# CristianSimion5/vk-raytracing-engine

Measured on AMD Instinct MI355X. Metric: Mrays/s, higher is better.
Workload: dtype f32

## Files before the change

### vk-raytracing-engine_amd/csrc/device_scene.h

```cpp
#pragma once
#include <hip/hip_runtime.h>
#include <stddef.h>
#include <stdint.h>
#include "../../include/vkrt_host_device.h"
#include "device_math.h"

struct DevInstance
{
  float o2w[12];
  float w2o[9];
  int32_t primMesh;
  uint32_t vis;
  int32_t pad;
};
static_assert(sizeof(DevInstance) == 96, "DevInstance");
#define VKRT_VIS_CULL_DISABLE 0x100u
#define VKRT_VIS_FLIP 0x200u
#define VKRT_VIS_MIRRORED 0x10000u

#define VKRT_VERTEX_QUADS 3
#define VKRT_VERTEX_BYTES 48u
struct DevTexRef
{
  uint32_t offset;
// ... 118 lines not shown
  uint32_t tilesX, tileCount;
  uint32_t tileFirst;
  float* image;
  unsigned int* workCounter;
  DevCounters* counters;
};

struct WfBuffers
{
  unsigned* ctrl;
  float4* planes;
  float4* stage;
  uint32_t capacity;
  uint32_t groups;
  float4* sampleState;
};
```

### vk-raytracing-engine_amd/csrc/kernels.h

```cpp
#pragma once
#include <hip/hip_runtime.h>
#include "device_scene.h"
#include "wf_schedule.h"

hipError_t vkrt_launch_pathtrace(const TraceParams& P, unsigned gridBlocks, bool count, hipStream_t stream);
int        vkrt_pathtrace_block_size();
hipError_t vkrt_pathtrace_occupancy(size_t ldsBytes, int* blocksPerCU);
hipError_t vkrt_launch_trace_rays(const DevScene& sc, unsigned n, const float* o, const float* d, float tmin, float tmax, int anyHit,
                                  float* t, float* u, float* v, int* gid, hipStream_t stream);
hipError_t vkrt_launch_eval_math(int op, unsigned n, const float* a, const float* b, float* out, hipStream_t stream);
#define VKRT_EVAL_SHADE_MAX_LIGHTS 16
hipError_t vkrt_launch_eval_shade(unsigned n, const float* in, float4* lights, float* out, hipStream_t stream);

hipError_t vkrt_launch_query(const DevQueryScene& sc, const float4* rays, uint64_t n, uint32_t seed, bool filter, bool opaque, bool alpha, float4* hits,
                             int* occ, hipStream_t stream);
hipError_t vkrt_launch_query_multi(const DevQueryScene& sc, const float4* rays, uint64_t n, uint32_t seed, bool filter, bool opaque, bool alpha,
                                   uint32_t maxHits, float4* hits, int* counts, hipStream_t stream);
hipError_t vkrt_launch_closest_point(const DevQueryScene& sc, const float4* queries, uint64_t n, bool filter, float4* hits, unsigned long long* work,
                                     hipStream_t stream);
hipError_t vkrt_launch_node_masks(const DevScene& sc, uint32_t nodeCount, uint32_t instCount, uint32_t sweeps, uint2* masks, hipStream_t stream);
hipError_t vkrt_launch_material_alpha(DevMaterial* table, uint32_t first, uint32_t count, const uint2* src, hipStream_t stream);
hipError_t vkrt_launch_hit_surface(const DevSurfaceScene& sc, const float4* hits, uint32_t n, bool material, float4* out, hipStream_t stream);

struct WfTiming
{
  hipEvent_t* events;
  int capacity;
  int used;
};
struct WfAsync
{
  hipStream_t streams[VKRT_WF_MAX_LANES];
  hipEvent_t fork, join[VKRT_WF_MAX_LANES];
  int count;
  hipEvent_t* pool;
  int poolSize;
};
size_t     vkrt_wf_state_bytes(uint32_t pathCapacity, int groups);
void       vkrt_wf_carve(void* base, uint32_t pathCapacity, int groups, WfBuffers* B);
struct WfOptions
{
  int subframes;
  int travBlock;
  int inFlight;
};
hipError_t vkrt_launch_wavefront(const TraceParams& P, const WfBuffers& B, const WfOptions& opt, int frames, uint32_t seedStep, bool count,
                                 hipStream_t stream, WfTiming* timing, const WfAsync* async);
void       vkrt_wf_launch_traverse(const TraceParams& P, const WfBuffers& B, int r, unsigned travBlock, bool count, dim3 tg, size_t tlds,
                                   hipStream_t stream);
void       vkrt_wf_launch_traverse_camera(const TraceParams& P, const WfBuffers& B, int r, int smpl, bool count, size_t tlds, hipStream_t stream);

struct HybridGi
{
  float4* color;
// ... 54 lines not shown
```

### vk-raytracing-engine_amd/csrc/vkrt_api.cpp

```cpp
#include <hip/hip_runtime.h>

#include <algorithm>
#include <chrono>
#include <cmath>
#include <cstdarg>
#include <cstdio>
#include <cstdlib>
#include <cstring>
#include <initializer_list>
#include <string>
#include <vector>

#include "../../include/vkrt.h"
#include "bvh_host.h"
#include "dev_buffer.h"
#include "device_scene.h"
#include "kernels.h"
#include "wide_node.h"

#define VKRT_TRI_THRESHOLD_DEFAULT 32
#define VKRT_WF_SHARE_DEFAULT 16
#define VKRT_WF_SHARE_FLAGS_DEFAULT 25
#define VKRT_WF_FRAMES_IN_FLIGHT_DEFAULT 3
#define VKRT_SPLIT_BUDGET_DEFAULT -1
// ... 37 lines not shown
  std::vector<uint32_t> indices;
  std::vector<vkrt_prim_mesh> primMeshes;
  std::vector<vkrt_node> nodes;
  uint32_t lightCount = 0, materialCount = 0;
  std::vector<float> materialAlpha;
  std::vector<void*> allocs;
  DevScene dev{};
  vkrt::TreeBuffers accel;
  bool built = false;
  vkrt_accel_info info{};
  unsigned int* workCounter = nullptr;
  DevCounters* counters = nullptr;
  hipEvent_t evStart = nullptr, evStop = nullptr;
  bool timed = false;
  void* wfMem = nullptr;
  WfBuffers wf{};
  WfAsync wfAsync{};
  std::vector<hipEvent_t> wfEvents;
  WfTiming wfTiming{};
  bool wfTimed = false;
  int splitResolved = 0;
  int wfTimingRounds = 0;
  std::vector<hipEvent_t> wfPool;
  int opt[VKRT_OPT_ALPHA_TEST + 1] = {0, 1, 1, 3, 64, VKRT_WF_SHARE_DEFAULT, VKRT_TRI_THRESHOLD_DEFAULT, 0, VKRT_WF_SHARE_FLAGS_DEFAULT, 1, 0, 0, 0,
                                            VKRT_WF_FRAMES_IN_FLIGHT_DEFAULT, VKRT_SPLIT_BUDGET_DEFAULT, VKRT_WF_SAMPLE_SYNC_DEFAULT, VKRT_WF_CAMERA_ROUNDS_DEFAULT,
                                      VKRT_WF_TRI_LEND_DEFAULT, 0};
  bool hasLargeTriangles = false;
  bool wavefront = true;
  bool stale = false;
  bool refitted = false;
// ... 212 lines not shown
{
  groups = std::max(1, std::min(VKRT_WF_MAX_LANES, groups));
  if(paths >= (1u << 28))
    return fail(VKRT_ERR_UNSUPPORTED, "wavefront mode: %u path records in one shard (limit 2^28 - 1: split the launch into shards)", paths);
  if(!s->wfMem || s->wf.capacity < paths || (int)s->wf.groups < groups)
  {
    HIP_TRY(hipStreamSynchronize(stream));
    if(s->wfMem) (void)hipFree(s->wfMem);
    s->wfMem = nullptr;
    paths = std::max(paths, s->wf.capacity);
    groups = std::max(groups, (int)s->wf.groups);
    s->wf = WfBuffers{};
    HIP_TRY(hipMalloc(&s->wfMem, vkrt_wf_state_bytes(paths, groups)));
    vkrt_wf_carve(s->wfMem, paths, groups, &s->wf);
  }
  if(s->wfAsync.count == 0)
  {
    HIP_TRY(hipEventCreateWithFlags(&s->wfAsync.fork, hipEventDisableTiming));
    for(int j = 0; j < VKRT_WF_MAX_LANES; j++)
    {
      HIP_TRY(hipStreamCreateWithFlags(&s->wfAsync.streams[j], hipStreamNonBlocking));
      HIP_TRY(hipEventCreateWithFlags(&s->wfAsync.join[j], hipEventDisableTiming));
    }
    s->wfAsync.count = VKRT_WF_MAX_LANES;
  }
  return VKRT_OK;
}

int ensureFrameCall(vkrt_scene* s, uint32_t tiles, uint32_t frames, hipStream_t stream)
{
// ... 432 lines not shown
  if(hipEventCreate(&s->evStart) != hipSuccess || hipEventCreate(&s->evStop) != hipSuccess)
    return bail(fail(VKRT_ERR_HIP, "hipEventCreate"));
  *out = s;
  return VKRT_OK;
}

void vkrt_scene_destroy(vkrt_scene* s)
{
  if(!s)
    return;
  (void)hipSetDevice(s->device);
  freeAccel(s);
  for(void* p : s->allocs)
    (void)hipFree(p);
  if(s->wfMem) (void)hipFree(s->wfMem);
  if(s->wfAsync.count)
  {
    (void)hipEventDestroy(s->wfAsync.fork);
    for(int j = 0; j < s->wfAsync.count; j++)
    {
      (void)hipStreamDestroy(s->wfAsync.streams[j]);
      (void)hipEventDestroy(s->wfAsync.join[j]);
    }
  }
  for(hipEvent_t e : s->wfEvents) (void)hipEventDestroy(e);
  for(hipEvent_t e : s->wfPool) (void)hipEventDestroy(e);
  if(s->evStart) (void)hipEventDestroy(s->evStart);
  if(s->evStop) (void)hipEventDestroy(s->evStop);
  delete s;
}
// ... 1431 lines not shown
```

### vk-raytracing-engine_amd/csrc/wavefront.hip

```cpp
#include <hip/hip_runtime.h>
#include <algorithm>
#include <cstdlib>
#include <cstring>

#include "device_math.h"
#include "device_scene.h"
#include "kernels.h"
#include "rgen.h"
#include "hybrid_gi.h"
#include "shade.h"
#include "traverse.h"
#include "traverse_wide.h"
#include "traverse_share.h"

#define WF_BLOCK 256
#define VKRT_FLAG_COUNT_WORK 2u

#include "wf_streams.h"

VKRT_DEV unsigned packFlags(const LaneState& L)
{
  return (L.prd.depth & 0xffu) | (((unsigned)L.smpl & 0xffffu) << 8) | ((L.prd.isSpecular ? 1u : 0u) << 25);
}

VKRT_DEV void loadCommon(const TraceParams& P, const WfBuffers& B, int parity, int type, unsigned i, LaneState& L)
{
  const float4 s0 = wfLoad(rec(B, parity, type, WF_S0, i)), s1 = wfLoad(rec(B, parity, type, WF_S1, i)), s2 = wfLoad(rec(B, parity, type, WF_S2, i));
  const unsigned flags = __float_as_uint(s1.w), pix = __float_as_uint(s2.w);
  L.curWeight = mk3(s0.x, s0.y, s0.z); L.prd.seed = __float_as_uint(s0.w);
  L.hitValue = mk3(s1.x, s1.y, s1.z);
  L.prd.depth = flags & 0xffu; L.smpl = (int)((flags >> 8) & 0xffffu);
  L.prd.isSpecular = ((flags >> 25) & 1u) != 0u;
  L.hitValues = mk3(s2.x, s2.y, s2.z);
// ... 33 lines not shown
VKRT_DEV int finishSegment(const TraceParams& P, const WfBuffers& B, LaneState& L, bool shadowHit, f3 contrib, f3 nextWeight)
{
  const SegmentStep step = stepSegment(P, L, shadowHit, contrib, nextWeight);
  if(step == SEG_SAMPLE_END)
  {
    if(P.flags & VKRT_FLAG_SAMPLE_SYNC)
    {
      wfStore(B.sampleState + pixelSlot(P, L.px, L.lrow), make_float4(L.hitValues.x, L.hitValues.y, L.hitValues.z, __uint_as_float(L.prd.seed)));
      return -1;
    }
    startSample(P, L);
  }
  return step == SEG_PIXEL_DONE ? -1 : WF_C;
}

VKRT_DEV unsigned claimSlots(const WfBuffers& B, int parity, int to, unsigned lane, unsigned* wsum)
{
  const unsigned wave = threadIdx.x >> 6, nw = blockDim.x >> 6;
  const unsigned long long m[WF_TYPES] = {__ballot(to == WF_C), __ballot(to == WF_S), __ballot(to == WF_P)};
  if(lane == 0)
  {
#pragma unroll
    for(int t = 0; t < WF_TYPES; t++) wsum[t * (nw + 1) + wave] = (unsigned)__popcll(m[t]);
  }
  __syncthreads();
  if(threadIdx.x < WF_TYPES)
  {
    unsigned* w = wsum + threadIdx.x * (nw + 1);
    unsigned tot = 0;
    for(unsigned k = 0; k < nw; k++)
    {
      const unsigned c = w[k];
      w[k] = tot;
      tot += c;
    }
    w[nw] = tot ? atomicAdd(countOf(B, parity, (int)threadIdx.x), tot) : 0u;
  }
  __syncthreads();
  if(to < 0)
    return 0u;
  const unsigned long long below = (1ull << lane) - 1ull;
  const unsigned long long mine = to == WF_C ? m[0] : to == WF_S ? m[1] : m[2];
  return wsum[to * (nw + 1) + nw] + wsum[to * (nw + 1) + wave] + (unsigned)__popcll(mine & below);
}

__global__ __launch_bounds__(WF_BLOCK) void k_wf_init(const TraceParams P, const WfBuffers B)
{
  const unsigned lane = lane_id();
  const unsigned w = blockIdx.x * blockDim.x + threadIdx.x;
  bool alive = false;
  unsigned nPixels = 0;
  LaneState L;
  uint32_t x, y, lrow;
  if(pixelOfWork(P, w, P.tileFirst, x, y, lrow))
  {
    startPixel(P, L, x, y, lrow);
    nPixels = 1;
    if(P.pc.samples <= 0 || P.pc.depth <= 0)
      storePixel(P, L);
    else
      alive = true;
  }
  __shared__ unsigned wsum[WF_TYPES * (WF_BLOCK / 64 + 1)];
  const unsigned slot = claimSlots(B, 0, alive ? WF_C : -1, lane, wsum);
  if(alive)
    storeClosest(B, 0, slot, L);
  __shared__ unsigned long long red[VKRT_COUNTER_STRIDE * (WF_BLOCK / 64)];
  const unsigned vals[6] = {0, 0, 0, 0, 0, nPixels};
  blockAddCounters(&P.counters->v[blockIdx.x % VKRT_COUNTER_SLOTS][0], vals, 6, red);
}

__global__ __launch_bounds__(WF_BLOCK) void k_wf_sample_init(const TraceParams P, const WfBuffers B, const int round, const int smpl)
{
  const unsigned lane = lane_id();
  const unsigned w = blockIdx.x * blockDim.x + threadIdx.x;
  bool alive = false;
  LaneState L;
  uint32_t x, y, lrow;
  if(pixelOfWork(P, w, P.tileFirst, x, y, lrow))
  {
    const float4 st = wfLoad(B.sampleState + pixelSlot(P, x, lrow));
    bindPixel(P, L, x, lrow);
    L.prd.seed = __float_as_uint(st.w);
    L.hitValues = mk3(st.x, st.y, st.z);
    L.smpl = smpl;
    startSample(P, L);
    alive = true;
  }
  __shared__ unsigned wsum[WF_TYPES * (WF_BLOCK / 64 + 1)];
  const unsigned slot = claimSlots(B, round & 1, alive ? WF_C : -1, lane, wsum);
  if(alive)
    storeClosest(B, round & 1, slot, L);
}

VKRT_DEV bool advanceSegmentHybrid(const TraceParams& P, const HybridGi& G, LaneState& L, bool shadowHit, f3 contrib, f3 nextWeight, float lightDist)
{
  L.stage = 0;
  if(giSegmentStep(P.pc, L.prd, L.curWeight, L.hitValue, L.hitValues.x, shadowHit, contrib, nextWeight, lightDist))
    return true;
  hybridStorePixel(P, G, (size_t)L.lrow * P.fullW + L.px, true, L.hitValue, L.hitValues.x, L.hitValues.y);
  return false;
}

struct ShadeLds
{
  float lut[512];
  unsigned wsum[WF_TYPES * (WF_BLOCK / 64 + 1)];
};

template <bool PAIR, bool HYBRID, bool CAMERA = false>
VKRT_DEV void shadeHitBlock(const TraceParams& P, const WfBuffers& B, const HybridGi& G, const int par, const unsigned count, const unsigned block, ShadeLds& lds,
                            const int smpl = 0)
{
  const int type = PAIR ? WF_P : WF_C;
  const unsigned lane = lane_id();
  const unsigned qi = block * WF_BLOCK + threadIdx.x;
  ShadeStats st = shadeStatsInit(P.sc, lds.lut);
  unsigned* wsum = lds.wsum;
  int to = -1;
  LaneState L;
  f3 contrib = mk3(0.0f), nextWeight = mk3(0.0f);
  uint32_t x = 0, y = 0, lrow = 0;
  if(CAMERA ? pixelOfWork(P, qi, P.tileFirst, x, y, lrow) : qi < count)
  {
    if(CAMERA)
    {
      bindPixel(P, L, x, lrow);
      if(smpl == 0)
      {
        L.prd.seed = pixelSeed(P, x, y);
        L.hitValues = mk3(0.0f);
      }
      else
      {
        const float4 s = wfLoad(B.sampleState + pixelSlot(P, x, lrow));
        L.prd.seed = __float_as_uint(s.w);
        L.hitValues = mk3(s.x, s.y, s.z);
      }
      L.smpl = smpl;
      startSample(P, L);
    }
    else
      loadCommon(P, B, par, type, qi, L);
    const float4 h = wfLoad(rec(B, par, type, WF_H0, qi)), t4 = wfLoad(rec(B, par, type, WF_H1, qi));
    if(!CAMERA)
    {
      const float4 rd = wfLoad(rec(B, par, type, PAIR ? WF_R2 : WF_R1, qi));
      L.prd.rayDirection = mk3(rd.x, rd.y, rd.z);
    }
    L.prd.rayOrigin = mk3(0.0f);
    if(PAIR)
    {
      const float4 s3 = wfLoad(rec(B, par, WF_P, WF_S3, qi));
      const bool shadowHit = __float_as_int(h.x) != 0;
      if(HYBRID)
        (void)advanceSegmentHybrid(P, G, L, shadowHit, mk3(s3.x, s3.y, s3.z), L.curWeight, L.prd.depth == 1u ? wfLoad(rec(B, par, WF_P, WF_R1, qi)).w : 0.0f);
      else
        (void)advanceSegment(P, L, shadowHit, mk3(s3.x, s3.y, s3.z), L.curWeight);
    }
    RayHit hit;
    hit.t = h.x; hit.u = h.y; hit.v = h.z; hit.slot = __float_as_int(h.w);
    const uint4 ts = make_uint4(__float_as_uint(t4.x), __float_as_uint(t4.y), __float_as_uint(t4.z), __float_as_uint(t4.w));
    if(hit.slot >= 0)
      closestHitShaderInst(P.sc, P.pc, hit, (uint32_t)hit.slot, ts, L.prd.rayDirection, L.prd, st);
    else
      missShader(P.pc, L.prd);
    segmentTerms(L.prd, L.curWeight, contrib, nextWeight);
    const bool dead = !HYBRID && (P.flags & VKRT_FLAG_SKIP_DEAD_SHADOW) != 0u && contrib.x == 0.0f && contrib.y == 0.0f && contrib.z == 0.0f;
    if(!L.prd.isSpecular && L.prd.depth != 100u && !dead)
      to = (L.prd.depth + 1u < (uint32_t)P.pc.depth) ? WF_P : WF_S;
    else if(HYBRID)
      to = advanceSegmentHybrid(P, G, L, false, contrib, nextWeight, 0.0f) ? WF_C : -1;
    else
      to = finishSegment(P, B, L, false, contrib, nextWeight);
  }
  const unsigned slot = claimSlots(B, par ^ 1, to, lane, wsum);
  if(to == WF_C)
    storeClosest(B, par ^ 1, slot, L);
  else if(to >= 0)
    storeShadow(B, par ^ 1, to, slot, L, contrib, nextWeight);
  if(P.flags & VKRT_FLAG_COUNT_WORK)
  {
    __shared__ unsigned long long red[VKRT_COUNTER_STRIDE * (WF_BLOCK / 64)];
    const unsigned vals[5] = {0, 0, st.hits, st.diffuse, st.taps};
    blockAddCounters(&P.counters->v[blockIdx.x % VKRT_COUNTER_SLOTS][0], vals, 5, red);
  }
}

template <bool HYBRID>
VKRT_DEV void shadeShadowBlock(const TraceParams& P, const WfBuffers& B, const HybridGi& G, const int par, const unsigned count, const unsigned block, ShadeLds& lds)
{
  const unsigned lane = lane_id();
  const unsigned qi = block * WF_BLOCK + threadIdx.x;
  unsigned* wsum = lds.wsum;
  bool toClosest = false;
  LaneState L;
  if(qi < count)
  {
    loadCommon(P, B, par, WF_S, qi, L);
    const float4 h = wfLoad(rec(B, par, WF_S, WF_H0, qi)), s3 = wfLoad(rec(B, par, WF_S, WF_S3, qi));
    L.prd.rayOrigin = mk3(0.0f);
    L.prd.rayDirection = mk3(0.0f);
    const bool shadowHit = __float_as_int(h.w) >= 0;
    if(HYBRID)
      toClosest = advanceSegmentHybrid(P, G, L, shadowHit, mk3(s3.x, s3.y, s3.z), L.curWeight, L.prd.depth == 1u ? wfLoad(rec(B, par, WF_S, WF_R1, qi)).w : 0.0f);
    else
      toClosest = finishSegment(P, B, L, shadowHit, mk3(s3.x, s3.y, s3.z), L.curWeight) == WF_C;
  }
  const unsigned slot = claimSlots(B, par ^ 1, toClosest ? WF_C : -1, lane, wsum);
  if(toClosest)
    storeClosest(B, par ^ 1, slot, L);
}

template <bool HYBRID>
VKRT_DEV void shadeRound(const TraceParams& P, const WfBuffers& B, const HybridGi& G, const int round)
{
  const int par = round & 1;
  const unsigned cC = *countOf(B, par, WF_C), cS = *countOf(B, par, WF_S), cP = *countOf(B, par, WF_P);
  const unsigned nC = (cC + WF_BLOCK - 1) / WF_BLOCK, nP = (cP + WF_BLOCK - 1) / WF_BLOCK, nS = (cS + WF_BLOCK - 1) / WF_BLOCK;
  unsigned blk = blockIdx.x;
  __shared__ ShadeLds lds;
  if(blk < nC)
    shadeHitBlock<false, HYBRID>(P, B, G, par, cC, blk, lds);
  else if((blk -= nC) < nP)
    shadeHitBlock<true, HYBRID>(P, B, G, par, cP, blk, lds);
  else if((blk -= nP) < nS)
    shadeShadowBlock<HYBRID>(P, B, G, par, cS, blk, lds);
}
__global__ __launch_bounds__(WF_BLOCK) void k_wf_shade(const TraceParams P, const WfBuffers B, const int round)
{
  const HybridGi none{};
  shadeRound<false>(P, B, none, round);
}
__global__ __launch_bounds__(WF_BLOCK) void k_wf_shade_hybrid(const TraceParams P, const WfBuffers B, const HybridGi G, const int round)
{
  shadeRound<true>(P, B, G, round);
}
__global__ __launch_bounds__(WF_BLOCK) void k_wf_shade_camera(const TraceParams P, const WfBuffers B, const int round, const int smpl)
{
  const HybridGi none{};
  __shared__ ShadeLds lds;
  shadeHitBlock<false, false, true>(P, B, none, round & 1, 0u, blockIdx.x, lds, smpl);
}

__global__ __launch_bounds__(WF_BLOCK) void k_hy_gi_init(const TraceParams P, const WfBuffers B, const HybridGi G, const uint2* tmp)
{
  const unsigned lane = lane_id();
  const unsigned w = blockIdx.x * blockDim.x + threadIdx.x;
  bool alive = false;
  LaneState L;
  uint32_t x, y, lrow;
  if(pixelOfWork(P, w, P.tileFirst, x, y, lrow))
  {
    const size_t p = (size_t)lrow * P.fullW + x;
    const GbufferPixel g = loadGbufferPixel(G, p);
    const uint2 t = tmp[p];
    const float alpha = __uint_as_float(t.y);
    if(g.shaded)
    {
      bindPixel(P, L, x, lrow);
      L.prd.seed = t.x;
      giFirstRay(P, g, L.prd, L.curWeight);
      L.hitValue = mk3(0.0f);
      L.hitValues = mk3(0.0f, alpha, 0.0f);
      L.smpl = 0;
      L.stage = 0;
      alive = L.prd.depth < (uint32_t)P.pc.depth;
    }
    if(!alive)
      hybridStorePixel(P, G, p, g.shaded, mk3(0.0f), 0.0f, alpha);
  }
  __shared__ unsigned wsum[WF_TYPES * (WF_BLOCK / 64 + 1)];
  const unsigned slot = claimSlots(B, 0, alive ? WF_C : -1, lane, wsum);
  if(alive)
    storeClosest(B, 0, slot, L);
}

__global__ __launch_bounds__(WF_BLOCK) void k_wf_blend(const TraceParams P, const float4* stage)
{
  uint32_t x, y, lrow;
  if(pixelOfWork(P, blockIdx.x * blockDim.x + threadIdx.x, P.tileFirst, x, y, lrow))
  {
    const size_t p = (size_t)lrow * P.fullW + x;
    blendPixel((float4*)P.image + p, stage[p], P.pc.frame);
  }
}

#define WF_CTRL_BYTES (256 * VKRT_WF_MAX_LANES)
size_t vkrt_wf_state_bytes(uint32_t pathCapacity, int groups)
{
  const size_t g = (size_t)std::max(groups, 1);
  return g * pathCapacity * 2 * WF_SLOTS * sizeof(float4) + (g > 1 ? g * pathCapacity * sizeof(float4) : 0) + g * pathCapacity * sizeof(float4) +
         WF_CTRL_BYTES;
}

void vkrt_wf_carve(void* base, uint32_t pathCapacity, int groups, WfBuffers* B)
{
  const size_t g = (size_t)std::max(groups, 1);
  char* p = (char*)base;
  B->ctrl = (unsigned*)p;
  p += WF_CTRL_BYTES;
  B->planes = (float4*)p;
  p += g * pathCapacity * 2 * WF_SLOTS * sizeof(float4);
  B->stage = g > 1 ? (float4*)p : nullptr;
  p += g > 1 ? g * pathCapacity * sizeof(float4) : 0;
  B->sampleState = (float4*)p;
  B->capacity = pathCapacity;
  B->groups = (uint32_t)g;
}

static unsigned pixelBlocks(const TraceParams& P) { return (P.tileCount * 64u + WF_BLOCK - 1) / WF_BLOCK; }
static hipError_t subframeBegin(const TraceParams& P, const WfBuffers& B, bool init, hipStream_t stream)
{
  const hipError_t e = hipMemsetAsync(B.ctrl, 0, 64, stream);
  if(e == hipSuccess && init)
    hipLaunchKernelGGL(k_wf_init, dim3(pixelBlocks(P)), dim3(WF_BLOCK), 0, stream, P, B);
  return e;
}
static void launchTraverse(const TraceParams& P, const WfBuffers& B, int r, unsigned travBlock, bool count, hipStream_t stream)
{
  const unsigned work = P.tileCount * 64u, tb = (travBlock == 256u || travBlock == 128u) ? travBlock : 64u;
  vkrt_wf_launch_traverse(P, B, r, tb, count, dim3(2 * ((work + tb - 1) / tb) + 4), (size_t)P.sc.stackCap * tb * sizeof(int), stream);
}
static void subframeRound(const TraceParams& P, const WfBuffers& B, int r, int cameraSample, unsigned travBlock, bool count, hipStream_t stream, WfTiming* timing)
{
  const bool timed = timing && timing->events && 2 * (timing->used + 1) <= timing->capacity;
  if(timed)
    (void)hipEventRecord(timing->events[2 * timing->used], stream);
  if(cameraSample >= 0)
    vkrt_wf_launch_traverse_camera(P, B, r, cameraSample, count, (size_t)P.sc.stackCap * 64u * sizeof(int), stream);
  else
    launchTraverse(P, B, r, travBlock, count, stream);
  if(timed)
  {
    (void)hipEventRecord(timing->events[2 * timing->used + 1], stream);
    timing->used++;
  }
  if(cameraSample >= 0)
    hipLaunchKernelGGL(k_wf_shade_camera, dim3(pixelBlocks(P)), dim3(WF_BLOCK), 0, stream, P, B, r, cameraSample);
  else
    hipLaunchKernelGGL(k_wf_shade, dim3(pixelBlocks(P) + 3), dim3(WF_BLOCK), 0, stream, P, B, r);
}

hipError_t vkrt_launch_wavefront(const TraceParams& P, const WfBuffers& B, const WfOptions& opt, int frames, uint32_t seedStep, bool count,
                                 hipStream_t stream, WfTiming* timing, const WfAsync* async)
{
  const WfCall call{P.pc.samples, P.pc.depth, (P.flags & VKRT_FLAG_SAMPLE_SYNC) != 0u, (P.flags & VKRT_FLAG_CAMERA_ROUNDS) != 0u, P.tileCount, frames,
                    opt.inFlight, opt.subframes, (int)B.groups, async ? async->count : 0, timing != nullptr};
  const WfLanes lanes = wfLanes(call);
  const int L = lanes.F * lanes.S;
  const bool staged = lanes.F > 1;
  if(staged && wfPoolEvents(lanes.frames) > async->poolSize)
    return hipErrorInvalidValue;
  hipStream_t laneStream[VKRT_WF_MAX_LANES];
  WfBuffers Bq[VKRT_WF_MAX_LANES];
  laneStream[0] = stream;
  Bq[0] = B;
  const size_t groupQuads = (size_t)2 * WF_SLOTS * B.capacity;
  for(int q = 0; L > 1 && q < L; q++)
  {
    const int g = q / lanes.S, j = q % lanes.S;
    const uint32_t tile0 = lanes.tileFirst(j);
    Bq[q].ctrl = B.ctrl + 64 * q;
    Bq[q].planes = B.planes + (size_t)g * groupQuads + (size_t)2 * WF_SLOTS * ((size_t)tile0 * 64u);
    Bq[q].stage = staged ? B.stage + (size_t)g * B.capacity : nullptr;
    Bq[q].sampleState = B.sampleState + (size_t)g * B.capacity;
    Bq[q].capacity = (lanes.tileFirst(j + 1) - tile0) * 64u;
    Bq[q].groups = 1;
    laneStream[q] = async->streams[q];
  }
  int forked = 0;
  auto joinLanes = [&]() {
    hipError_t first = hipSuccess;
    for(int q = 0; q < forked; q++)
    {
      hipError_t x = hipEventRecord(async->join[q], laneStream[q]);
      if(x == hipSuccess) x = hipStreamWaitEvent(stream, async->join[q], 0);
      if(x != hipSuccess)
// ... 56 lines not shown
    e = hipErrorUnknown;
  const hipError_t ej = joinLanes();
  if(e == hipSuccess) e = ej;
  if(e == hipSuccess) e = hipGetLastError();
  return e;
}

uint2* vkrt_wf_hybrid_tmp(const WfBuffers& B)
{
  return (uint2*)(B.planes + (size_t)(1 * WF_SLOTS + 0) * B.capacity);
}

hipError_t vkrt_launch_hybrid_gi(const TraceParams& P, const WfBuffers& B, const HybridGi& G, unsigned travBlock, hipStream_t stream)
{
  const unsigned work = P.tileCount * 64u;
  hipError_t e = hipMemsetAsync(B.ctrl, 0, 64, stream);
  if(e != hipSuccess)
    return e;
  const unsigned blocks = (work + WF_BLOCK - 1) / WF_BLOCK;
  hipLaunchKernelGGL(k_hy_gi_init, dim3(blocks), dim3(WF_BLOCK), 0, stream, P, B, G, (const uint2*)vkrt_wf_hybrid_tmp(B));
  const int rounds = P.pc.depth;
  for(int r = 0; r < rounds; r++)
  {
    launchTraverse(P, B, r, travBlock, false, stream);
    hipLaunchKernelGGL(k_wf_shade_hybrid, dim3(blocks + 3), dim3(WF_BLOCK), 0, stream, P, B, G, r);
  }
  return hipGetLastError();
}
```

### vk-raytracing-engine_amd/csrc/wf_streams.h

```cpp
#pragma once
#include <hip/hip_runtime.h>

#include "device_math.h"
#include "device_scene.h"
#include "traverse_wide.h"

#define WF_PLANES 9
#define WF_TYPES 3
enum { WF_R0 = 0, WF_R1, WF_R2, WF_H0, WF_H1, WF_S0, WF_S1, WF_S2, WF_S3 };
enum { WF_C = 0, WF_S = 1, WF_P = 2 };

#define WF_SLOTS_CS 8
#define WF_SLOTS (WF_SLOTS_CS + WF_PLANES)
VKRT_DEV float4* plane(const WfBuffers& B, int parity, int type, int k)
{
  const int slot = type == WF_P ? WF_SLOTS_CS + k : (k > WF_R2 ? k - 1 : k);
  return B.planes + ((size_t)(parity * WF_SLOTS + slot)) * B.capacity;
}
VKRT_DEV unsigned* countOf(const WfBuffers& B, int parity, int type) { return &B.ctrl[parity * 4 + type]; }
VKRT_DEV float4* rec(const WfBuffers& B, int parity, int type, int k, unsigned i)
{
  return (float4*)((char*)plane(B, parity, type, k) + (size_t)((type == WF_S ? B.capacity - 1u - i : i) * 16u));
}

VKRT_DEV float4 wfLoad(const float4* p)
{
  const vkrt_v4f v = __builtin_nontemporal_load((const vkrt_v4f*)p);
  return make_float4(v.x, v.y, v.z, v.w);
}
VKRT_DEV void wfStore(float4* p, float4 v) { *p = v; }
```

### vk-raytracing-engine_amd/csrc/wf_traverse.hip

```cpp
#include <hip/hip_runtime.h>

#include "device_math.h"
#include "device_scene.h"
#include "kernels.h"
#include "rgen.h"
#include "traverse.h"
#include "traverse_wide.h"
#include "traverse_share.h"
#include "wf_streams.h"

enum { WF_K_CLOSEST_C = 0, WF_K_CLOSEST_P = 1, WF_K_SHADOW_S = 2, WF_K_SHADOW_P = 3 };

VKRT_DEV void storeHit(const TraceParams& P, const WfBuffers& B, int par, int kind, unsigned qi, const RayHit& hit)
{
  if(kind == WF_K_SHADOW_S)
    wfStore(rec(B, par, WF_S, WF_H0, qi), make_float4(0.0f, 0.0f, 0.0f, __int_as_float(hit.slot >= 0 ? 0 : -1)));
  else if(kind == WF_K_SHADOW_P)
    ((float*)rec(B, par, WF_P, WF_H0, qi))[0] = __int_as_float(hit.slot >= 0 ? 1 : 0);
  else
  {
    const int type = kind == WF_K_CLOSEST_C ? WF_C : WF_P;
    int inst = -1;
    if(hit.slot >= 0)
    {
// ... 6 lines not shown
      wfStore(rec(B, par, WF_C, WF_H0, qi), make_float4(hit.t, hit.u, hit.v, __int_as_float(inst)));
    else
    {
      h[1] = hit.u; h[2] = hit.v; h[3] = __int_as_float(inst);
    }
  }
}

template <bool COUNT, bool WIDE, int TB, int TM = 0>
__global__ __launch_bounds__(TB)
__attribute__((amdgpu_waves_per_eu(TM != 0 && WIDE && TB == 64 ? (COUNT && (TM & VKRT_TM_ALPHA) != 0 ? 4 : 5) : 1)))
void k_wf_traverse(const TraceParams P, const WfBuffers B, const int round)
{
  extern __shared__ int lds_stack[];
  const int par = round & 1;
  const unsigned cC = *countOf(B, par, WF_C), cS = *countOf(B, par, WF_S), cP = *countOf(B, par, WF_P);
  if(blockIdx.x == 0 && threadIdx.x == 0)
  {
    for(int t = 0; t < WF_TYPES; t++) *countOf(B, par ^ 1, t) = 0u;
    if(cC + cP) atomicAdd(&P.counters->v[round % VKRT_COUNTER_SLOTS][0], (unsigned long long)cC + cP);
    if(cS + cP) atomicAdd(&P.counters->v[round % VKRT_COUNTER_SLOTS][1], (unsigned long long)cS + cP);
    if(cP) atomicAdd(&P.counters->v[round % VKRT_COUNTER_SLOTS][11], (unsigned long long)cP);
  }
  const unsigned nC = (cC + TB - 1) / TB, nP = (cP + TB - 1) / TB, nS = (cS + TB - 1) / TB;
  unsigned blk = blockIdx.x;
  int kind;
  unsigned count;
  if(blk < nC) { kind = WF_K_CLOSEST_C; count = cC; }
  else if((blk -= nC) < nP) { kind = WF_K_CLOSEST_P; count = cP; }
  else if((blk -= nP) < nS) { kind = WF_K_SHADOW_S; count = cS; }
  else if((blk -= nS) < nP) { kind = WF_K_SHADOW_P; count = cP; }
  else return;
  const bool anyHit = kind >= WF_K_SHADOW_S;
  const int type = kind == WF_K_CLOSEST_C ? WF_C : kind == WF_K_SHADOW_S ? WF_S : WF_P;
  const unsigned qi = blk * TB + threadIdx.x;
  const bool valid = qi < count;
  float4 r0 = make_float4(0.0f, 0.0f, 0.0f, 0.0f), r1 = make_float4(1.0f, 0.0f, 0.0f, 0.0f);
  if(valid)
  {
    r0 = wfLoad(rec(B, par, type, WF_R0, qi));
    r1 = wfLoad(rec(B, par, type, kind == WF_K_CLOSEST_P ? WF_R2 : WF_R1, qi));
    if(kind == WF_K_CLOSEST_P)
      r0.w = 10000.0f;
  }
  uint32_t raySeed = 0u;
  if((TM & VKRT_TM_DISSOLVE) && valid)
    raySeed = __float_as_uint(wfLoad(rec(B, par, type, WF_S0, qi)).w);
  TravCount tc;
  __shared__ int shareLds[VKRT_SHARE_LDS_WORDS];
  RayHit hit;
  if(WIDE && TB == 64 && P.sc.shareMinIdle != 0u && P.sc.triThreshold != 0u)
// ... 15 lines not shown
  {
    __shared__ unsigned long long red[VKRT_COUNTER_STRIDE * (TB / 64)];
    const unsigned vals[10] = {0, 0, 0, 0, 0, 0, tc.nodes, tc.tris, tc.waveNodeSteps, tc.waveTriSteps};
    blockAddCounters(&P.counters->v[blockIdx.x % VKRT_COUNTER_SLOTS][0], vals, 10, red);
  }
}

template <bool COUNT, int TM>
__global__ __launch_bounds__(64)
__attribute__((amdgpu_waves_per_eu(TM != 0 ? 5 : 1)))
void k_wf_traverse_camera(const TraceParams P, const WfBuffers B, const int round, const int smpl)
{
  extern __shared__ int lds_stack[];
  const int par = round & 1;
  if(blockIdx.x == 0 && threadIdx.x == 0)
    for(int t = 0; t < WF_TYPES; t++) *countOf(B, par ^ 1, t) = 0u;
  const unsigned w = blockIdx.x * 64u + threadIdx.x;
  uint32_t x = 0, y = 0, lrow = 0;
  const bool valid = pixelOfWork(P, w, P.tileFirst, x, y, lrow);
  f3 o = mk3(0.0f), d = mk3(1.0f, 0.0f, 0.0f);
  uint32_t raySeed = 0u;
  if(valid)
  {
    LaneState L;
    bindPixel(P, L, x, lrow);
    L.prd.seed = smpl == 0 ? pixelSeed(P, x, y) : __float_as_uint(((const float*)(B.sampleState + pixelSlot(P, x, lrow)))[3]);
    L.smpl = smpl;
    startSample(P, L);
    o = L.prd.rayOrigin; d = L.prd.rayDirection;
    raySeed = L.prd.seed;
  }
// ... 56 lines not shown
```

Before: 5445.

## Shard wavefront queue counters into per-segment heads to cut atomic contention

Replaces the single global per-type queue counters with WF_SEGMENTS (8) independent segment heads, each padded to its own cache-line stride. Producer blocks map to segments by block index and claim slots within that segment's region of the path buffers. Traverse and shade grids are re-sized so each segment is covered by interleaved blocks. This is meant to reduce contention on the global atomic counters. In exchange, the grids are larger and blocks can sit idle when segments are unevenly filled, and locality shifts within the record planes.

Result: no change. 5494 (median of 6 runs) (+0.9%).

```diff
diff --git a/vk-raytracing-engine_amd/csrc/device_scene.h b/vk-raytracing-engine_amd/csrc/device_scene.h
--- a/vk-raytracing-engine_amd/csrc/device_scene.h
+++ b/vk-raytracing-engine_amd/csrc/device_scene.h
@@ -156,4 +156,5 @@
   uint32_t capacity;
   uint32_t groups;
   float4* sampleState;
+  unsigned* heads;
 };
diff --git a/vk-raytracing-engine_amd/csrc/kernels.h b/vk-raytracing-engine_amd/csrc/kernels.h
--- a/vk-raytracing-engine_amd/csrc/kernels.h
+++ b/vk-raytracing-engine_amd/csrc/kernels.h
@@ -38,6 +38,7 @@
 };
 size_t     vkrt_wf_state_bytes(uint32_t pathCapacity, int groups);
 void       vkrt_wf_carve(void* base, uint32_t pathCapacity, int groups, WfBuffers* B);
+size_t     vkrt_wf_head_bytes();
 struct WfOptions
 {
   int subframes;
diff --git a/vk-raytracing-engine_amd/csrc/vkrt_api.cpp b/vk-raytracing-engine_amd/csrc/vkrt_api.cpp
--- a/vk-raytracing-engine_amd/csrc/vkrt_api.cpp
+++ b/vk-raytracing-engine_amd/csrc/vkrt_api.cpp
@@ -75,6 +75,7 @@
   hipEvent_t evStart = nullptr, evStop = nullptr;
   bool timed = false;
   void* wfMem = nullptr;
+  unsigned* wfHeads = nullptr;
   WfBuffers wf{};
   WfAsync wfAsync{};
   std::vector<hipEvent_t> wfEvents;
@@ -317,6 +318,9 @@
     HIP_TRY(hipMalloc(&s->wfMem, vkrt_wf_state_bytes(paths, groups)));
     vkrt_wf_carve(s->wfMem, paths, groups, &s->wf);
   }
+  if(!s->wfHeads)
+    HIP_TRY(hipMalloc((void**)&s->wfHeads, vkrt_wf_head_bytes()));
+  s->wf.heads = s->wfHeads;
   if(s->wfAsync.count == 0)
   {
     HIP_TRY(hipEventCreateWithFlags(&s->wfAsync.fork, hipEventDisableTiming));
@@ -779,6 +783,7 @@
   for(void* p : s->allocs)
     (void)hipFree(p);
   if(s->wfMem) (void)hipFree(s->wfMem);
+  if(s->wfHeads) (void)hipFree(s->wfHeads);
   if(s->wfAsync.count)
   {
     (void)hipEventDestroy(s->wfAsync.fork);
diff --git a/vk-raytracing-engine_amd/csrc/wavefront.hip b/vk-raytracing-engine_amd/csrc/wavefront.hip
--- a/vk-raytracing-engine_amd/csrc/wavefront.hip
+++ b/vk-raytracing-engine_amd/csrc/wavefront.hip
@@ -17,6 +17,7 @@
 #define VKRT_FLAG_COUNT_WORK 2u
 
 #include "wf_streams.h"
+static_assert(WF_BLOCK == WF_SEG_BLOCK, "the segments are sized for producer workgroups of WF_SEG_BLOCK work items");
 
 VKRT_DEV unsigned packFlags(const LaneState& L)
 {
@@ -80,7 +81,7 @@
   return step == SEG_PIXEL_DONE ? -1 : WF_C;
 }
 
-VKRT_DEV unsigned claimSlots(const WfBuffers& B, int parity, int to, unsigned lane, unsigned* wsum)
+VKRT_DEV unsigned claimSlots(const WfBuffers& B, const WfSeg& seg, int parity, int to, unsigned lane, unsigned* wsum)
 {
   const unsigned wave = threadIdx.x >> 6, nw = blockDim.x >> 6;
   const unsigned long long m[WF_TYPES] = {__ballot(to == WF_C), __ballot(to == WF_S), __ballot(to == WF_P)};
@@ -100,14 +101,14 @@
       w[k] = tot;
       tot += c;
     }
-    w[nw] = tot ? atomicAdd(countOf(B, parity, (int)threadIdx.x), tot) : 0u;
+    w[nw] = tot ? atomicAdd(countOf(B, seg.g, parity, (int)threadIdx.x), tot) : 0u;
   }
   __syncthreads();
   if(to < 0)
     return 0u;
   const unsigned long long below = (1ull << lane) - 1ull;
   const unsigned long long mine = to == WF_C ? m[0] : to == WF_S ? m[1] : m[2];
-  return wsum[to * (nw + 1) + nw] + wsum[to * (nw + 1) + wave] + (unsigned)__popcll(mine & below);
+  return slotOf(seg, to, wsum[to * (nw + 1) + nw] + wsum[to * (nw + 1) + wave] + (unsigned)__popcll(mine & below));
 }
 
 __global__ __launch_bounds__(WF_BLOCK) void k_wf_init(const TraceParams P, const WfBuffers B)
@@ -128,7 +129,7 @@
       alive = true;
   }
   __shared__ unsigned wsum[WF_TYPES * (WF_BLOCK / 64 + 1)];
-  const unsigned slot = claimSlots(B, 0, alive ? WF_C : -1, lane, wsum);
+  const unsigned slot = claimSlots(B, segOf(B, wfSegOfBlock(blockIdx.x)), 0, alive ? WF_C : -1, lane, wsum);
   if(alive)
     storeClosest(B, 0, slot, L);
   __shared__ unsigned long long red[VKRT_COUNTER_STRIDE * (WF_BLOCK / 64)];
@@ -154,7 +155,7 @@
     alive = true;
   }
   __shared__ unsigned wsum[WF_TYPES * (WF_BLOCK / 64 + 1)];
-  const unsigned slot = claimSlots(B, round & 1, alive ? WF_C : -1, lane, wsum);
+  const unsigned slot = claimSlots(B, segOf(B, wfSegOfBlock(blockIdx.x)), round & 1, alive ? WF_C : -1, lane, wsum);
   if(alive)
     storeClosest(B, round & 1, slot, L);
 }
@@ -175,12 +176,13 @@
 };
 
 template <bool PAIR, bool HYBRID, bool CAMERA = false>
-VKRT_DEV void shadeHitBlock(const TraceParams& P, const WfBuffers& B, const HybridGi& G, const int par, const unsigned count, const unsigned block, ShadeLds& lds,
-                            const int smpl = 0)
+VKRT_DEV void shadeHitBlock(const TraceParams& P, const WfBuffers& B, const HybridGi& G, const WfSeg& seg, const int par, const unsigned count,
+                            const unsigned chunk, ShadeLds& lds, const int smpl = 0)
 {
   const int type = PAIR ? WF_P : WF_C;
   const unsigned lane = lane_id();
-  const unsigned qi = block * WF_BLOCK + threadIdx.x;
+  const unsigned qi = chunk * WF_BLOCK + threadIdx.x;
+  const unsigned slot = CAMERA ? qi : slotOf(seg, type, qi);
   ShadeStats st = shadeStatsInit(P.sc, lds.lut);
   unsigned* wsum = lds.wsum;
   int to = -1;
@@ -207,20 +209,20 @@
       startSample(P, L);
     }
     else
-      loadCommon(P, B, par, type, qi, L);
-    const float4 h = wfLoad(rec(B, par, type, WF_H0, qi)), t4 = wfLoad(rec(B, par, type, WF_H1, qi));
+      loadCommon(P, B, par, type, slot, L);
+    const float4 h = wfLoad(rec(B, par, type, WF_H0, slot)), t4 = wfLoad(rec(B, par, type, WF_H1, slot));
     if(!CAMERA)
     {
-      const float4 rd = wfLoad(rec(B, par, type, PAIR ? WF_R2 : WF_R1, qi));
+      const float4 rd = wfLoad(rec(B, par, type, PAIR ? WF_R2 : WF_R1, slot));
       L.prd.rayDirection = mk3(rd.x, rd.y, rd.z);
     }
     L.prd.rayOrigin = mk3(0.0f);
     if(PAIR)
     {
-      const float4 s3 = wfLoad(rec(B, par, WF_P, WF_S3, qi));
+      const float4 s3 = wfLoad(rec(B, par, WF_P, WF_S3, slot));
       const bool shadowHit = __float_as_int(h.x) != 0;
       if(HYBRID)
-        (void)advanceSegmentHybrid(P, G, L, shadowHit, mk3(s3.x, s3.y, s3.z), L.curWeight, L.prd.depth == 1u ? wfLoad(rec(B, par, WF_P, WF_R1, qi)).w : 0.0f);
+        (void)advanceSegmentHybrid(P, G, L, shadowHit, mk3(s3.x, s3.y, s3.z), L.curWeight, L.prd.depth == 1u ? wfLoad(rec(B, par, WF_P, WF_R1, slot)).w : 0.0f);
       else
         (void)advanceSegment(P, L, shadowHit, mk3(s3.x, s3.y, s3.z), L.curWeight);
     }
@@ -240,11 +242,11 @@
     else
       to = finishSegment(P, B, L, false, contrib, nextWeight);
   }
-  const unsigned slot = claimSlots(B, par ^ 1, to, lane, wsum);
+  const unsigned next = claimSlots(B, seg, par ^ 1, to, lane, wsum);
   if(to == WF_C)
-    storeClosest(B, par ^ 1, slot, L);
+    storeClosest(B, par ^ 1, next, L);
   else if(to >= 0)
-    storeShadow(B, par ^ 1, to, slot, L, contrib, nextWeight);
+    storeShadow(B, par ^ 1, to, next, L, contrib, nextWeight);
   if(P.flags & VKRT_FLAG_COUNT_WORK)
   {
     __shared__ unsigned long long red[VKRT_COUNTER_STRIDE * (WF_BLOCK / 64)];
@@ -254,44 +256,47 @@
 }
 
 template <bool HYBRID>
-VKRT_DEV void shadeShadowBlock(const TraceParams& P, const WfBuffers& B, const HybridGi& G, const int par, const unsigned count, const unsigned block, ShadeLds& lds)
+VKRT_DEV void shadeShadowBlock(const TraceParams& P, const WfBuffers& B, const HybridGi& G, const WfSeg& seg, const int par, const unsigned count, const unsigned chunk,
+                               ShadeLds& lds)
 {
   const unsigned lane = lane_id();
-  const unsigned qi = block * WF_BLOCK + threadIdx.x;
+  const unsigned qi = chunk * WF_BLOCK + threadIdx.x;
+  const unsigned slot = slotOf(seg, WF_S, qi);
   unsigned* wsum = lds.wsum;
   bool toClosest = false;
   LaneState L;
   if(qi < count)
   {
-    loadCommon(P, B, par, WF_S, qi, L);
-    const float4 h = wfLoad(rec(B, par, WF_S, WF_H0, qi)), s3 = wfLoad(rec(B, par, WF_S, WF_S3, qi));
+    loadCommon(P, B, par, WF_S, slot, L);
+    const float4 h = wfLoad(rec(B, par, WF_S, WF_H0, slot)), s3 = wfLoad(rec(B, par, WF_S, WF_S3, slot));
     L.prd.rayOrigin = mk3(0.0f);
     L.prd.rayDirection = mk3(0.0f);
     const bool shadowHit = __float_as_int(h.w) >= 0;
     if(HYBRID)
-      toClosest = advanceSegmentHybrid(P, G, L, shadowHit, mk3(s3.x, s3.y, s3.z), L.curWeight, L.prd.depth == 1u ? wfLoad(rec(B, par, WF_S, WF_R1, qi)).w : 0.0f);
+      toClosest = advanceSegmentHybrid(P, G, L, shadowHit, mk3(s3.x, s3.y, s3.z), L.curWeight, L.prd.depth == 1u ? wfLoad(rec(B, par, WF_S, WF_R1, slot)).w : 0.0f);
     else
       toClosest = finishSegment(P, B, L, shadowHit, mk3(s3.x, s3.y, s3.z), L.curWeight) == WF_C;
   }
-  const unsigned slot = claimSlots(B, par ^ 1, toClosest ? WF_C : -1, lane, wsum);
+  const unsigned next = claimSlots(B, seg, par ^ 1, toClosest ? WF_C : -1, lane, wsum);
   if(toClosest)
-    storeClosest(B, par ^ 1, slot, L);
+    storeClosest(B, par ^ 1, next, L);
 }
 
 template <bool HYBRID>
 VKRT_DEV void shadeRound(const TraceParams& P, const WfBuffers& B, const HybridGi& G, const int round)
 {
   const int par = round & 1;
-  const unsigned cC = *countOf(B, par, WF_C), cS = *countOf(B, par, WF_S), cP = *countOf(B, par, WF_P);
-  const unsigned nC = (cC + WF_BLOCK - 1) / WF_BLOCK, nP = (cP + WF_BLOCK - 1) / WF_BLOCK, nS = (cS + WF_BLOCK - 1) / WF_BLOCK;
-  unsigned blk = blockIdx.x;
+  const WfSeg seg = segOf(B, wfSegOfBlock(blockIdx.x));
+  const unsigned cC = *countOf(B, seg.g, par, WF_C), cS = *countOf(B, seg.g, par, WF_S), cP = *countOf(B, seg.g, par, WF_P);
+  unsigned chunk = wfChunkOfBlock(blockIdx.x);
+  const int type = wfShadeKind(chunk, cC, cS, cP);
   __shared__ ShadeLds lds;
-  if(blk < nC)
-    shadeHitBlock<false, HYBRID>(P, B, G, par, cC, blk, lds);
-  else if((blk -= nC) < nP)
-    shadeHitBlock<true, HYBRID>(P, B, G, par, cP, blk, lds);
-  else if((blk -= nP) < nS)
-    shadeShadowBlock<HYBRID>(P, B, G, par, cS, blk, lds);
+  if(type == WF_C)
+    shadeHitBlock<false, HYBRID>(P, B, G, seg, par, cC, chunk, lds);
+  else if(type == WF_P)
+    shadeHitBlock<true, HYBRID>(P, B, G, seg, par, cP, chunk, lds);
+  else if(type == WF_S)
+    shadeShadowBlock<HYBRID>(P, B, G, seg, par, cS, chunk, lds);
 }
 __global__ __launch_bounds__(WF_BLOCK) void k_wf_shade(const TraceParams P, const WfBuffers B, const int round)
 {
@@ -306,7 +311,7 @@
 {
   const HybridGi none{};
   __shared__ ShadeLds lds;
-  shadeHitBlock<false, false, true>(P, B, none, round & 1, 0u, blockIdx.x, lds, smpl);
+  shadeHitBlock<false, false, true>(P, B, none, segOf(B, wfSegOfBlock(blockIdx.x)), round & 1, 0u, blockIdx.x, lds, smpl);
 }
 
 __global__ __launch_bounds__(WF_BLOCK) void k_hy_gi_init(const TraceParams P, const WfBuffers B, const HybridGi G, const uint2* tmp)
@@ -337,7 +342,7 @@
       hybridStorePixel(P, G, p, g.shaded, mk3(0.0f), 0.0f, alpha);
   }
   __shared__ unsigned wsum[WF_TYPES * (WF_BLOCK / 64 + 1)];
-  const unsigned slot = claimSlots(B, 0, alive ? WF_C : -1, lane, wsum);
+  const unsigned slot = claimSlots(B, segOf(B, wfSegOfBlock(blockIdx.x)), 0, alive ? WF_C : -1, lane, wsum);
   if(alive)
     storeClosest(B, 0, slot, L);
 }
@@ -353,6 +358,7 @@
 }
 
 #define WF_CTRL_BYTES (256 * VKRT_WF_MAX_LANES)
+size_t vkrt_wf_head_bytes() { return (size_t)VKRT_WF_MAX_LANES * WF_HEAD_WORDS * sizeof(unsigned); }
 size_t vkrt_wf_state_bytes(uint32_t pathCapacity, int groups)
 {
   const size_t g = (size_t)std::max(groups, 1);
@@ -378,7 +384,7 @@
 static unsigned pixelBlocks(const TraceParams& P) { return (P.tileCount * 64u + WF_BLOCK - 1) / WF_BLOCK; }
 static hipError_t subframeBegin(const TraceParams& P, const WfBuffers& B, bool init, hipStream_t stream)
 {
-  const hipError_t e = hipMemsetAsync(B.ctrl, 0, 64, stream);
+  const hipError_t e = hipMemsetAsync(B.heads, 0, WF_HEAD_WORDS * sizeof(unsigned), stream);
   if(e == hipSuccess && init)
     hipLaunchKernelGGL(k_wf_init, dim3(pixelBlocks(P)), dim3(WF_BLOCK), 0, stream, P, B);
   return e;
@@ -386,7 +392,7 @@
 static void launchTraverse(const TraceParams& P, const WfBuffers& B, int r, unsigned travBlock, bool count, hipStream_t stream)
 {
   const unsigned work = P.tileCount * 64u, tb = (travBlock == 256u || travBlock == 128u) ? travBlock : 64u;
-  vkrt_wf_launch_traverse(P, B, r, tb, count, dim3(2 * ((work + tb - 1) / tb) + 4), (size_t)P.sc.stackCap * tb * sizeof(int), stream);
+  vkrt_wf_launch_traverse(P, B, r, tb, count, dim3(wfTraverseGrid(work, tb)), (size_t)P.sc.stackCap * tb * sizeof(int), stream);
 }
 static void subframeRound(const TraceParams& P, const WfBuffers& B, int r, int cameraSample, unsigned travBlock, bool count, hipStream_t stream, WfTiming* timing)
 {
@@ -405,7 +411,7 @@
   if(cameraSample >= 0)
     hipLaunchKernelGGL(k_wf_shade_camera, dim3(pixelBlocks(P)), dim3(WF_BLOCK), 0, stream, P, B, r, cameraSample);
   else
-    hipLaunchKernelGGL(k_wf_shade, dim3(pixelBlocks(P) + 3), dim3(WF_BLOCK), 0, stream, P, B, r);
+    hipLaunchKernelGGL(k_wf_shade, dim3(wfShadeGrid(P.tileCount * 64u)), dim3(WF_BLOCK), 0, stream, P, B, r);
 }
 
 hipError_t vkrt_launch_wavefront(const TraceParams& P, const WfBuffers& B, const WfOptions& opt, int frames, uint32_t seedStep, bool count,
@@ -428,6 +434,7 @@
     const int g = q / lanes.S, j = q % lanes.S;
     const uint32_t tile0 = lanes.tileFirst(j);
     Bq[q].ctrl = B.ctrl + 64 * q;
+    Bq[q].heads = B.heads + (size_t)WF_HEAD_WORDS * q;
     Bq[q].planes = B.planes + (size_t)g * groupQuads + (size_t)2 * WF_SLOTS * ((size_t)tile0 * 64u);
     Bq[q].stage = staged ? B.stage + (size_t)g * B.capacity : nullptr;
     Bq[q].sampleState = B.sampleState + (size_t)g * B.capacity;
@@ -514,7 +521,7 @@
 hipError_t vkrt_launch_hybrid_gi(const TraceParams& P, const WfBuffers& B, const HybridGi& G, unsigned travBlock, hipStream_t stream)
 {
   const unsigned work = P.tileCount * 64u;
-  hipError_t e = hipMemsetAsync(B.ctrl, 0, 64, stream);
+  hipError_t e = hipMemsetAsync(B.heads, 0, WF_HEAD_WORDS * sizeof(unsigned), stream);
   if(e != hipSuccess)
     return e;
   const unsigned blocks = (work + WF_BLOCK - 1) / WF_BLOCK;
@@ -523,7 +530,7 @@
   for(int r = 0; r < rounds; r++)
   {
     launchTraverse(P, B, r, travBlock, false, stream);
-    hipLaunchKernelGGL(k_wf_shade_hybrid, dim3(blocks + 3), dim3(WF_BLOCK), 0, stream, P, B, G, r);
+    hipLaunchKernelGGL(k_wf_shade_hybrid, dim3(wfShadeGrid(work)), dim3(WF_BLOCK), 0, stream, P, B, G, r);
   }
   return hipGetLastError();
 }
diff --git a/vk-raytracing-engine_amd/csrc/wf_segments.h b/vk-raytracing-engine_amd/csrc/wf_segments.h
--- /dev/null
+++ b/vk-raytracing-engine_amd/csrc/wf_segments.h
@@ -0,0 +1,56 @@
+#pragma once
+#include <cstdint>
+
+#ifndef WF_SEGMENTS
+#define WF_SEGMENTS 8
+#endif
+#define WF_SEG_BLOCK 256
+#define WF_HEAD_STRIDE 32
+#define WF_HEAD_WORDS (WF_SEGMENTS * WF_HEAD_STRIDE)
+
+#if defined(__HIPCC__)
+#define WF_SEG_FN __host__ __device__ inline
+#else
+#define WF_SEG_FN inline
+#endif
+
+WF_SEG_FN uint32_t wfSegBlocks(uint32_t work) { return (work + WF_SEG_BLOCK - 1u) / WF_SEG_BLOCK; }
+WF_SEG_FN uint32_t wfSegTailGap(uint32_t cap) { return wfSegBlocks(cap) * WF_SEG_BLOCK - cap; }
+WF_SEG_FN uint32_t wfSegOfBlock(uint32_t block) { return block % WF_SEGMENTS; }
+WF_SEG_FN uint32_t wfChunkOfBlock(uint32_t block) { return block / WF_SEGMENTS; }
+WF_SEG_FN uint32_t wfSegBlockCount(uint32_t cap, uint32_t g) { return (wfSegBlocks(cap) + WF_SEGMENTS - 1u - g) / WF_SEGMENTS; }
+WF_SEG_FN uint32_t wfSegCapacity(uint32_t cap, uint32_t g)
+{
+  const uint32_t nb = wfSegBlocks(cap);
+  return wfSegBlockCount(cap, g) * WF_SEG_BLOCK - ((nb > 0u && (nb - 1u) % WF_SEGMENTS == g) ? wfSegTailGap(cap) : 0u);
+}
+WF_SEG_FN uint32_t wfSegBase(uint32_t cap, uint32_t g)
+{
+  const uint32_t nb = wfSegBlocks(cap), q = nb / WF_SEGMENTS, r = nb % WF_SEGMENTS;
+  return (g * q + (g < r ? g : r)) * WF_SEG_BLOCK - ((nb > 0u && (nb - 1u) % WF_SEGMENTS < g) ? wfSegTailGap(cap) : 0u);
+}
+WF_SEG_FN uint32_t wfSegRecord(uint32_t base, uint32_t segCap, int type, uint32_t i) { return type == 1 ? base + segCap - 1u - i : base + i; }
+WF_SEG_FN int wfSegStep(int type) { return type == 1 ? -1 : 1; }
+WF_SEG_FN uint32_t wfHeadWord(uint32_t g, int parity, int type) { return g * WF_HEAD_STRIDE + (uint32_t)(parity * 4 + type); }
+
+WF_SEG_FN int wfTraverseKind(uint32_t& chunk, uint32_t tb, uint32_t cC, uint32_t cS, uint32_t cP)
+{
+  const uint32_t nC = (cC + tb - 1u) / tb, nP = (cP + tb - 1u) / tb, nS = (cS + tb - 1u) / tb;
+  if(chunk < nC) return 0;
+  if((chunk -= nC) < nP) return 1;
+  if((chunk -= nP) < nS) return 2;
+  if((chunk -= nS) < nP) return 3;
+  return -1;
+}
+WF_SEG_FN int wfShadeKind(uint32_t& chunk, uint32_t cC, uint32_t cS, uint32_t cP)
+{
+  const uint32_t nC = (cC + WF_SEG_BLOCK - 1u) / WF_SEG_BLOCK, nP = (cP + WF_SEG_BLOCK - 1u) / WF_SEG_BLOCK, nS = (cS + WF_SEG_BLOCK - 1u) / WF_SEG_BLOCK;
+  if(chunk < nC) return 0;
+  if((chunk -= nC) < nP) return 2;
+  if((chunk -= nP) < nS) return 1;
+  return -1;
+}
+
+WF_SEG_FN uint32_t wfSegMaxRecords(uint32_t work) { return (wfSegBlocks(work) + WF_SEGMENTS - 1u) / WF_SEGMENTS * WF_SEG_BLOCK; }
+WF_SEG_FN uint32_t wfShadeGrid(uint32_t work) { return WF_SEGMENTS * (wfSegMaxRecords(work) / WF_SEG_BLOCK + 2u); }
+WF_SEG_FN uint32_t wfTraverseGrid(uint32_t work, uint32_t tb) { return WF_SEGMENTS * (2u * (wfSegMaxRecords(work) / tb) + 4u); }
diff --git a/vk-raytracing-engine_amd/csrc/wf_streams.h b/vk-raytracing-engine_amd/csrc/wf_streams.h
--- a/vk-raytracing-engine_amd/csrc/wf_streams.h
+++ b/vk-raytracing-engine_amd/csrc/wf_streams.h
@@ -4,6 +4,7 @@
 #include "device_math.h"
 #include "device_scene.h"
 #include "traverse_wide.h"
+#include "wf_segments.h"
 
 #define WF_PLANES 9
 #define WF_TYPES 3
@@ -17,10 +18,16 @@
   const int slot = type == WF_P ? WF_SLOTS_CS + k : (k > WF_R2 ? k - 1 : k);
   return B.planes + ((size_t)(parity * WF_SLOTS + slot)) * B.capacity;
 }
-VKRT_DEV unsigned* countOf(const WfBuffers& B, int parity, int type) { return &B.ctrl[parity * 4 + type]; }
-VKRT_DEV float4* rec(const WfBuffers& B, int parity, int type, int k, unsigned i)
+struct WfSeg
 {
-  return (float4*)((char*)plane(B, parity, type, k) + (size_t)((type == WF_S ? B.capacity - 1u - i : i) * 16u));
+  unsigned g, base, cap;
+};
+VKRT_DEV WfSeg segOf(const WfBuffers& B, unsigned g) { return {g, wfSegBase(B.capacity, g), wfSegCapacity(B.capacity, g)}; }
+VKRT_DEV unsigned slotOf(const WfSeg& s, int type, unsigned i) { return wfSegRecord(s.base, s.cap, type, i); }
+VKRT_DEV unsigned* countOf(const WfBuffers& B, unsigned g, int parity, int type) { return &B.heads[wfHeadWord(g, parity, type)]; }
+VKRT_DEV float4* rec(const WfBuffers& B, int parity, int type, int k, unsigned slot)
+{
+  return (float4*)((char*)plane(B, parity, type, k) + (size_t)(slot * 16u));
 }
 
 VKRT_DEV float4 wfLoad(const float4* p)
diff --git a/vk-raytracing-engine_amd/csrc/wf_traverse.hip b/vk-raytracing-engine_amd/csrc/wf_traverse.hip
--- a/vk-raytracing-engine_amd/csrc/wf_traverse.hip
+++ b/vk-raytracing-engine_amd/csrc/wf_traverse.hip
@@ -44,27 +44,29 @@
 {
   extern __shared__ int lds_stack[];
   const int par = round & 1;
-  const unsigned cC = *countOf(B, par, WF_C), cS = *countOf(B, par, WF_S), cP = *countOf(B, par, WF_P);
-  if(blockIdx.x == 0 && threadIdx.x == 0)
+  const WfSeg seg = segOf(B, wfSegOfBlock(blockIdx.x));
+  const unsigned cC = *countOf(B, seg.g, par, WF_C), cS = *countOf(B, seg.g, par, WF_S), cP = *countOf(B, seg.g, par, WF_P);
+  if(threadIdx.x == 0)
   {
-    for(int t = 0; t < WF_TYPES; t++) *countOf(B, par ^ 1, t) = 0u;
-    if(cC + cP) atomicAdd(&P.counters->v[round % VKRT_COUNTER_SLOTS][0], (unsigned long long)cC + cP);
-    if(cS + cP) atomicAdd(&P.counters->v[round % VKRT_COUNTER_SLOTS][1], (unsigned long long)cS + cP);
-    if(cP) atomicAdd(&P.counters->v[round % VKRT_COUNTER_SLOTS][11], (unsigned long long)cP);
+    if(blockIdx.x == 0)
+      for(unsigned g = 0; g < WF_SEGMENTS; g++)
+        for(int t = 0; t < WF_TYPES; t++) *countOf(B, g, par ^ 1, t) = 0u;
+    if(blockIdx.x < WF_SEGMENTS)
+    {
+      if(cC + cP) atomicAdd(&P.counters->v[round % VKRT_COUNTER_SLOTS][0], (unsigned long long)cC + cP);
+      if(cS + cP) atomicAdd(&P.counters->v[round % VKRT_COUNTER_SLOTS][1], (unsigned long long)cS + cP);
+      if(cP) atomicAdd(&P.counters->v[round % VKRT_COUNTER_SLOTS][11], (unsigned long long)cP);
+    }
   }
-  const unsigned nC = (cC + TB - 1) / TB, nP = (cP + TB - 1) / TB, nS = (cS + TB - 1) / TB;
-  unsigned blk = blockIdx.x;
-  int kind;
-  unsigned count;
-  if(blk < nC) { kind = WF_K_CLOSEST_C; count = cC; }
-  else if((blk -= nC) < nP) { kind = WF_K_CLOSEST_P; count = cP; }
-  else if((blk -= nP) < nS) { kind = WF_K_SHADOW_S; count = cS; }
-  else if((blk -= nS) < nP) { kind = WF_K_SHADOW_P; count = cP; }
-  else return;
+  unsigned chunk = wfChunkOfBlock(blockIdx.x);
+  const int kind = wfTraverseKind(chunk, TB, cC, cS, cP);
+  if(kind < 0)
+    return;
+  const unsigned count = kind == WF_K_CLOSEST_C ? cC : kind == WF_K_SHADOW_S ? cS : cP;
   const bool anyHit = kind >= WF_K_SHADOW_S;
   const int type = kind == WF_K_CLOSEST_C ? WF_C : kind == WF_K_SHADOW_S ? WF_S : WF_P;
-  const unsigned qi = blk * TB + threadIdx.x;
-  const bool valid = qi < count;
+  const bool valid = chunk * TB + threadIdx.x < count;
+  const unsigned qi = slotOf(seg, type, chunk * TB) + (unsigned)(wfSegStep(type) * (int)threadIdx.x);
   float4 r0 = make_float4(0.0f, 0.0f, 0.0f, 0.0f), r1 = make_float4(1.0f, 0.0f, 0.0f, 0.0f);
   if(valid)
   {
@@ -110,7 +112,8 @@
   extern __shared__ int lds_stack[];
   const int par = round & 1;
   if(blockIdx.x == 0 && threadIdx.x == 0)
-    for(int t = 0; t < WF_TYPES; t++) *countOf(B, par ^ 1, t) = 0u;
+    for(unsigned g = 0; g < WF_SEGMENTS; g++)
+      for(int t = 0; t < WF_TYPES; t++) *countOf(B, g, par ^ 1, t) = 0u;
   const unsigned w = blockIdx.x * 64u + threadIdx.x;
   uint32_t x = 0, y = 0, lrow = 0;
   const bool valid = pixelOfWork(P, w, P.tileFirst, x, y, lrow);
```
